# empymod/emg3d

Hardware: AMD Instinct MI355X
Metric: Mcells/s per multigrid cycle (higher is better)
Workload: dtype c128

## Files before the change

### emg3d_amd/_lib.py

```python
import ctypes
import os

import numpy as np

_HERE = os.path.dirname(os.path.abspath(__file__))
LIB_PATH = os.environ.get("EMG3D_HIP_LIB") or os.path.join(_HERE, "libemg3d_hip.so")
LAB_PATH = os.path.join(_HERE, "libemg3d_hip_lab.so")

c_i64 = ctypes.c_int64
c_int = ctypes.c_int
c_vp = ctypes.c_void_p
c_double = ctypes.c_double
c_dp = ctypes.POINTER(ctypes.c_double)

ABI_VERSION = 104

SIGNATURES = {
    "emg3d_hip_version": (c_int, []),
    "emg3d_hip_device_count": (c_int, [ctypes.POINTER(c_int)]),
    "emg3d_hip_set_device": (c_int, [c_int]),
    "emg3d_hip_device_info": (c_int, [c_int, ctypes.c_char_p, ctypes.POINTER(c_i64), ctypes.POINTER(c_int)]),
    "emg3d_hip_mem_info": (c_int, [c_int, ctypes.POINTER(c_i64), ctypes.POINTER(c_i64)]),
    "emg3d_hip_release_cached": (c_i64, []),
    "emg3d_hip_cached_bytes": (c_i64, []),
    "emg3d_hip_cached_bytes_on": (c_i64, [c_int]),
    "emg3d_mg_placement": (c_int, [c_vp, c_int, ctypes.POINTER(c_int), ctypes.POINTER(c_int), ctypes.POINTER(ctypes.c_float)]),
    "emg3d_amat_x": (c_int, [c_int, c_i64, c_i64, c_i64, c_vp, c_vp, c_vp, c_vp, c_vp, c_vp, c_vp, c_vp, c_vp]),
    "emg3d_get_h_field": (c_int, [c_int, c_i64, c_i64, c_i64, c_vp, c_vp, c_vp, c_vp, c_vp, c_vp, c_double, c_double]),
    "emg3d_gauss_seidel": (c_int, [c_int, c_int, c_i64, c_i64, c_i64, c_vp, c_vp, c_vp, c_vp, c_vp, c_vp,
                                   c_vp, c_vp, c_vp, c_int, c_int]),
    "emg3d_restrict": (c_int, [c_int, c_i64, c_i64, c_i64, c_i64, c_i64, c_i64, c_vp, c_vp, c_vp, c_int]),
    "emg3d_restrict_weights": (c_int, [c_vp, c_vp, c_vp, c_i64, c_vp, c_vp, c_vp, c_i64, c_vp, c_vp, c_vp]),
    "emg3d_solve": (c_int, [c_int, c_vp, c_vp, c_i64]),
    "emg3d_blocks_to_amat": (c_int, [c_int, c_vp, c_vp, c_i64, c_vp, c_vp, c_vp, c_i64, c_i64]),
    "emg3d_prolongation": (c_int, [c_int, c_i64, c_i64, c_i64, c_vp, c_vp, c_vp, c_vp, c_vp, c_vp, c_int]),
    "emg3d_restrict_model": (c_int, [c_int, c_i64, c_i64, c_i64, c_vp, c_vp, c_int]),
    "emg3d_sweep_plan": (c_int, [c_int, c_i64, c_i64, c_i64, c_int, c_int, c_int, c_int, ctypes.c_char_p, ctypes.POINTER(c_i64)]),
    "emg3d_mg_create": (c_int, [ctypes.POINTER(c_vp), c_int, c_i64, c_i64, c_i64, c_vp, c_vp, c_vp, c_vp,
                                c_vp, c_vp, c_vp, c_vp, c_int]),
    "emg3d_mg_destroy": (None, [c_vp]),
    "emg3d_mg_create_sv": (c_int, [ctypes.POINTER(c_vp), c_int, c_i64, c_i64, c_i64, c_vp, c_vp, c_vp, c_vp,
                                   c_vp, c_vp, c_vp, c_vp, c_double, c_double, c_int]),
    "emg3d_mg_create_vs": (c_int, [ctypes.POINTER(c_vp), c_int, c_i64, c_i64, c_i64, c_vp, c_vp, c_vp, c_vp,
                                   c_vp, c_vp, c_vp, c_vp, c_vp, c_double, c_double, c_int, c_int]),
    "emg3d_mg_create_vse": (c_int, [ctypes.POINTER(c_vp), c_int, c_i64, c_i64, c_i64, c_vp, c_vp, c_vp, c_vp,
                                    c_vp, c_vp, c_vp, c_vp, c_vp, c_vp, c_double, c_double, c_double, c_int, c_int]),
    "emg3d_mg_set_smu0_eps": (c_int, [c_vp, c_double, c_double, c_double]),
    "emg3d_mg_set_sfield_vector": (c_int, [c_vp, c_vp, c_double, c_double]),
    "emg3d_mg_set_sfield_dipole": (c_int, [c_vp, c_vp, c_vp, c_int, c_int, c_vp]),
    "emg3d_source_field": (c_int, [c_int, c_i64, c_i64, c_i64, c_vp, c_vp, c_vp, c_vp, c_vp, c_vp, c_int, c_vp, c_vp]),
    "emg3d_mg_prepare": (c_int, [c_vp, c_int, c_int]),
    "emg3d_mg_set_trace": (c_int, [c_vp, c_int]),
# ... 133 lines not shown
    return {"name": name.value.decode(), "total_mem": mem.value, "cu_count": cus.value}


def mem_info(device=0):
    fr, tot = c_i64(0), c_i64(0)
    check(load().emg3d_hip_mem_info(device, ctypes.byref(fr), ctypes.byref(tot)), "emg3d_hip_mem_info")
    return {"free": fr.value, "total": tot.value, "pooled": int(load().emg3d_hip_cached_bytes()),
            "pooled_on_device": int(load().emg3d_hip_cached_bytes_on(device))}


def sweep_plan(vnC, direction, dtype=np.complex128, ordering='colour', nsys=1, cu_count=0):
    name = ctypes.create_string_buffer(64)
    info = (c_i64 * 6)()
    check(load().emg3d_sweep_plan(dtype_code(dtype), int(vnC[0]), int(vnC[1]), int(vnC[2]), int(direction),
                                  1 if ordering == 'colour' else 0, int(nsys), int(cu_count), name, info), "emg3d_sweep_plan")
    return {"kernel": name.value.decode(), "lines_per_colour": info[0], "lines_per_wave": info[1], "rounds": info[2],
            "factor_kind": info[3], "split": bool(info[4]), "big_offsets": bool(info[5])}
```

### emg3d_amd/csrc/emg3d_hip.hip

```cpp
#include "../../include/emg3d_hip.h"

#include <cstring>
#include <new>

#include <chrono>
#include "mg.hpp"
#include "receivers.hpp"
#include "source.hpp"
#include "gradient.hpp"
#include "regrid.hpp"

#define EMG3D_HIP_VERSION EMG3D_HIP_ABI_VERSION

namespace {

template <class T>
MG<T>* as(emg3d_mg_t* mg) { return static_cast<MG<T>*>(reinterpret_cast<emg3d_mg*>(mg)); }

static int current_device() { int d = 0; if (hipGetDevice(&d) != hipSuccess) { (void)hipGetLastError(); d = 0; } return d; }

template <class T> static T scalar_of(double re, double im);
template <> double scalar_of<double>(double re, double) { return re; }
template <> c128 scalar_of<c128>(double re, double im) { return mk(re, im); }

// ... 481 lines not shown
    if (cu_count > 0) {
        m.cu_count = cu_count;
        m.tha_lds_state = 1; m.tha_lds_limit = 160 * 1024;
    } else m.device = current_device();
    m.order = order; m.nsys = nsys;
    m.lv0 = std::make_shared<Level<T>>();
    Level<T>& L = *m.lv0;
    L.nC[0] = nx; L.nC[1] = ny; L.nC[2] = nz;
    MG<T>::shape_level(L);
    i64 inf[6];
    m.plan_sweep(L, dir - 1, name, inf);
    for (int k = 0; k < 6; ++k) info[k] = inf[k];
    return 0;
}

extern "C" {

int emg3d_hip_version(void) { return EMG3D_HIP_VERSION; }

int64_t emg3d_hip_release_cached(void) { return (int64_t)DevicePool::get().release_all(); }
int64_t emg3d_hip_cached_bytes(void) { return (int64_t)DevicePool::get().bytes_held(); }
int64_t emg3d_hip_cached_bytes_on(int device) { return device < 0 ? 0 : (int64_t)DevicePool::get().bytes_held_on(device); }

int emg3d_hip_device_count(int* count) {
    HIP_TRY(hipGetDeviceCount(count));
    return 0;
}

int emg3d_hip_set_device(int device) {
    HIP_TRY(hipSetDevice(device));
// ... 76 lines not shown
    return dtype ? prolong_impl<c128>(nx, ny, nz, hx, hy, hz, origin, e, ce, sc_dir)
                 : prolong_impl<double>(nx, ny, nz, hx, hy, hz, origin, e, ce, sc_dir);
}

int emg3d_restrict_model(int is_complex, int64_t nx, int64_t ny, int64_t nz, void* cparam, const void* param,
                         int sc_dir) {
    return is_complex ? restrict_model_impl<c128>(nx, ny, nz, cparam, param, sc_dir)
                      : restrict_model_impl<double>(nx, ny, nz, cparam, param, sc_dir);
}

int emg3d_sweep_plan(int dtype, int64_t nx, int64_t ny, int64_t nz, int dir, int order, int nsys, int cu_count, char* name,
                     int64_t* info) {
    if (nx < 2 || ny < 2 || nz < 2 || dir < 1 || dir > 3 || order < 0 || order > 1 || nsys < 1 || nsys > 64 || !name || !info) return -2;
    return dtype ? sweep_plan_impl<c128>(nx, ny, nz, dir, order, nsys, cu_count, name, info)
                 : sweep_plan_impl<double>(nx, ny, nz, dir, order, nsys, cu_count, name, info);
}

int emg3d_mg_create(emg3d_mg_t** out, int dtype, int64_t nx, int64_t ny, int64_t nz, const double* hx,
                    const double* hy, const double* hz, const double* origin, const void* eta_x,
                    const void* eta_y, const void* eta_z, const double* zeta, int device) {
    if (!out) return -1;
    return dtype ? create_impl<c128>(out, 1, nx, ny, nz, hx, hy, hz, origin, eta_x, eta_y, eta_z, zeta, device)
                 : create_impl<double>(out, 0, nx, ny, nz, hx, hy, hz, origin, eta_x, eta_y, eta_z, zeta, device);
}

int emg3d_mg_create_sv(emg3d_mg_t** out, int dtype, int64_t nx, int64_t ny, int64_t nz, const double* hx,
                       const double* hy, const double* hz, const double* origin, const double* sv_x,
                       const double* sv_y, const double* sv_z, const double* zeta, double smu0_re,
                       double smu0_im, int device) {
    if (!out || !sv_x) return -1;
// ... 557 lines not shown
```

### emg3d_amd/csrc/mg.hpp

```cpp
#pragma once
#include <algorithm>
#include <cmath>
#include <cstdlib>
#include <cstring>
#include <map>
#include <memory>
#include <mutex>
#include <chrono>
#include <vector>

#include "common.hpp"
#include "smooth.hpp"
#include "stencil.hpp"
#include "smooth_qpl.hpp"
#include "smooth_qc.hpp"
#include "smooth_thm.hpp"
#include "smooth_tha.hpp"
#include "sweep_launch.hpp"

template <class T>
struct Level {
    i64 nC[3];
    i64 nE, nCells;
    FieldLayout fl;
// ... 6 lines not shown
    unsigned char* sflag[3] = {nullptr, nullptr, nullptr};
    bool sflag_valid[3] = {false, false, false};
    bool s_dense = false;
    bool zeta_sep = false;
    T *s = nullptr, *e = nullptr, *r = nullptr;
    T *eT = nullptr, *sT = nullptr;
    T* etaT[3] = {nullptr, nullptr, nullptr};
    double* zetaT = nullptr;
    bool sT_valid = false;
    FieldLayout flT;
    CellLayout clT;
    T *eW[2] = {nullptr, nullptr}, *sW[2] = {nullptr, nullptr};
    double* zetaW[2] = {nullptr, nullptr};
    bool sW_valid[2] = {false, false};
    int e_home = 0;
    T* fac[3] = {nullptr, nullptr, nullptr};
    void* qd[3][4] = {{nullptr, nullptr, nullptr, nullptr}, {nullptr, nullptr, nullptr, nullptr}, {nullptr, nullptr, nullptr, nullptr}};
    unsigned qdn[3][4] = {{0, 0, 0, 0}, {0, 0, 0, 0}, {0, 0, 0, 0}};
    i64 fac_lines[3] = {0, 0, 0};
    i64 fac_mid[3] = {0, 0, 0};
    int fac_kind[3] = {0, 0, 0};
};

struct Transfer {
    int sc = -1;
    int co[3] = {0, 0, 0};
    double* w[3][3] = {{nullptr, nullptr, nullptr}, {nullptr, nullptr, nullptr}, {nullptr, nullptr, nullptr}};
    int* pidx[3] = {nullptr, nullptr, nullptr};
    double* pwt[3] = {nullptr, nullptr, nullptr};
};
// ... 898 lines not shown
        a.xcd = xcd_map;
        a.tile = q_tile;
        {
            const int ax[3] = {a.L, a.P, a.Q};
            a.rs.ihL = a.ih[a.L]; a.rs.ihP = a.ih[a.P]; a.rs.ihQ = a.ih[a.Q];
            a.rs.hL = a.h[a.L]; a.rs.hP = a.h[a.P]; a.rs.hQ = a.h[a.Q];
            a.rs.nL = (unsigned)a.nC[a.L]; a.rs.slot0 = 0;
            a.rs.nP = (unsigned)a.nC[a.P]; a.rs.nQ = (unsigned)a.nC[a.Q];
            a.rs.csL = (unsigned)a.cl.st[a.L]; a.rs.csP = (unsigned)a.cl.st[a.P]; a.rs.csQ = (unsigned)a.cl.st[a.Q];
            for (int c = 0; c < 3; ++c) {
                a.rs.off[c] = (unsigned)a.fl.off[ax[c]];
                for (int d = 0; d < 3; ++d) a.rs.st[c][d] = (unsigned)a.fl.st[ax[c]][ax[d]];
            }
        }
        a.qd = nullptr; a.qdn = 0;
        a.qpl = 0; a.qM = 0; a.seg = 0; a.qlpw = 0;
        if (qpl(L, dir)) { int NW, M, seg; qpl_shape(L.nC[a.L], NW, M, seg); a.qpl = NW; a.qM = M; a.seg = seg; }
        a.tha = tha_helpers(L, dir);
        a.mode = 0; a.cP = a.cQ = 0; a.cntA = a.cntB = 0; a.t = a.jQ0 = a.cnt = 0;
        a.bt = sweep ? batch(L) : Batch();
    }

    bool q_on(const LineArgs<T>& a) const {
        return use_q >= 2 || (use_q == 1 && a.nA[0] * a.nB2[0] >= q_min_lines());
    }
    bool thm_on(const Level<T>& L, const LineArgs<T>& a) const { return twist_ok(L, a); }
    bool twist_ok(const Level<T>& L, const LineArgs<T>& a) const {
        if (q_on(a)) return false;
        if (!use_twist || !rp_fits(L) || L.nC[a.L] < 3) return false;
        const i64 nQ = L.nC[a.Q];
// ... 360 lines not shown
            L.eW[w] = cands[best];
            block_tag[cands[best]] = 1 + w;
            for (int k = 0; k < R.tries; ++k) if (k != best) release(cands[k]);
            moved |= best != 0;
            if (getenv("EMG3D_LOG_SETUP")) {
                fprintf(stderr, "[place] working copy %d (%s-lines, %.0f MB): kept candidate %d of %d;", w, dir == 0 ? "x" : dir == 1 ? "y" : "z",
                        (double)n * sizeof(T) / 1048576.0, best, R.tries);
                for (int k = 0; k < R.tries; ++k) fprintf(stderr, " %.3f", R.ms[k]);
                fprintf(stderr, " ms per sweep\n");
            }
        }
        if (moved) drop_graphs();
        check_launch();
    }

    void smooth_line(Level<T>& L, int dir, int nu, bool conv_in = true, bool conv_out = true) {
        if (nu <= 0) return;
        ensure_factor(L, dir);
        ensure_qdesc(L, dir);
        if (dry) { prepare_work(L, dir); return; }
        if (conv_in) to_work(L, dir);
        ensure_sflags(L, dir);
        LineArgs<T> a;
        line_args(L, dir, a, true);
        const bool big = q_big(L) && !rp_fits(L);
        const bool rp = rp_fits(L) || big;
        const i64 nP = L.nC[a.P], nQ = L.nC[a.Q];
        const i64 nB[2] = {(nQ - 0) / 2, (nQ - 1) / 2};
        int iback = 0;
        int last_c = -1;
        for (int it = 0; it < nu; ++it) {
            iback = 1 - iback;
            if (order == 1) {
                for (int ch = 0; ch < 4; ++ch) {
                    const int c = iback ? colour_perm_b[ch] : colour_perm[ch];
                    if (skip_idempotent && c == last_c) continue;
                    last_c = c;
                    a.mode = 0; a.cP = c & 1; a.cQ = c >> 1;
                    a.cntA = a.nA[a.cP]; a.cntB = nB[a.cQ];
                    a.rs.slot0 = (unsigned)a.base[c];
                    a.qd = L.qd[dir][c]; a.qdn = (L.qd[dir][c] ? L.qdn[dir][c] : 0u);
                    const i64 n = a.cntA * a.cntB;
                    if (n <= 0) continue;
// ... 62 lines not shown
                                       dim3(EMG_LINE_BLOCK), 0, stream, a);
                }
            }
        }
        if (hl) convert_field(L, L.eW[1], L.e, 1, true);
        check_launch();
    }

    void smoothing(Level<T>& L, int nu, int lr_dir) {
        const int lr = current_lr_dir(lr_dir, L.nC);
        if (lr == 0) smooth_point(L, nu);
        int dirs[3], nd = 0;
        if (lr == 1 || lr == 5 || lr == 6 || lr == 7) dirs[nd++] = 0;
        if (lr == 2 || lr == 4 || lr == 6 || lr == 7) dirs[nd++] = 1;
        if (lr == 3 || lr == 4 || lr == 5 || lr == 7) dirs[nd++] = 2;
        for (int k = 0; k < nd; ++k) {
            const bool in = (k == 0) || work_id(L, dirs[k - 1]) != work_id(L, dirs[k]);
            const bool out = (k == nd - 1) || work_id(L, dirs[k + 1]) != work_id(L, dirs[k]);
            smooth_line(L, dirs[k], nu, in, out);
        }
    }

    void residual(Level<T>& L, int mode, int slot) {
        ResidualArgs<T> a;
        for (int q = 0; q < 3; ++q) { a.nC[q] = L.nC[q]; a.eta[q] = L.eta[q]; a.h[q] = L.h[q]; a.ih[q] = L.ih[q]; }
        a.fl = L.fl; a.r = L.r; a.s = L.s; a.e = L.e; a.zeta = L.zeta; a.bt = batch(L);
        if (!dry && L.e_home == 1) {
            if (!L.sW_valid[1]) { convert_field(L, L.sW[1], L.s, 1, true); L.sW_valid[1] = true; }
            a.e = L.eW[1]; a.s = L.sW[1]; a.xs = 1;
        }
        const i64 plane = (L.nC[0] + 1) * (L.nC[1] + 1);
        const i64 cells = L.nC[0] * L.nC[1] * L.nC[2];
        const int kz = cells < res_zm_min ? 1 : res_kz ? res_kz : (cells * nsys >= ((i64)8 << 20) ? 8 : 4);
        const i64 nNz = L.nC[2] + 1;
// ... 209 lines not shown
```

### emg3d_amd/csrc/smooth.hpp

```cpp
#pragma once
#include "common.hpp"

#define EMG_LINE_BLOCK 64

template <class T>
struct LineArgs {
    int L, P, Q;
    i64 nC[3];
    FieldLayout fl;
    CellLayout cl;
    T* e;
    const T* s;
    const T* eta[3];
    const double* zeta;
    const double* h[3];
    const double* ih[3];
    int split;
    i64 mid;
    int xcd;
    int tile;
    struct Resolved {
        const double *ihL, *ihP, *ihQ;
        const double *hL, *hP, *hQ;
        unsigned nL, csL, csP, csQ;
// ... 5 lines not shown
    int qm;
    int qpl;
    int qM, seg;
    const unsigned char* sflag;
    int zsep;
    int qlpw;
    int tha;
    int fcomp;
    T* fac;
    const void* qd;
    unsigned qdn;
    i64 nLinesTot;
    i64 base[4];
    i64 nA[2];
    i64 nB2[2];
    int mode;
    int cP, cQ;
    i64 cntA, cntB;
    i64 t, jQ0, cnt;
};

template <class T>
__device__ __forceinline__ bool line_of_thread(const LineArgs<T>& a, i64& jP, i64& jQ) {
    const i64 idx = (i64)blockIdx.x * blockDim.x + threadIdx.x;
    if (a.mode == 0) {
        if (idx >= a.cntA * a.cntB) return false;
        const i64 b = idx / a.cntA, q = idx - b * a.cntA;
        jP = 1 + a.cP + 2 * q;
        jQ = 1 + a.cQ + 2 * b;
    } else {
// ... 1165 lines not shown
```

### emg3d_amd/csrc/smooth_qpl.hpp

```cpp
#pragma once
#include "smooth.hpp"


template <int K>
__device__ __forceinline__ double quad_bcast(double v) {
    constexpr int ctrl = K | (K << 2) | (K << 4) | (K << 6);
    int lo = __double2loint(v), hi = __double2hiint(v);
    lo = __builtin_amdgcn_update_dpp(0, lo, ctrl, 0xf, 0xf, false);
    hi = __builtin_amdgcn_update_dpp(0, hi, ctrl, 0xf, 0xf, false);
    return __hiloint2double(hi, lo);
}
template <int K>
__device__ __forceinline__ c128 quad_bcast(c128 v) { return mk(quad_bcast<K>(v.re), quad_bcast<K>(v.im)); }
__device__ __forceinline__ double quad_sum(double v) {
    int lo = __double2loint(v), hi = __double2hiint(v);
    double o = __hiloint2double(__builtin_amdgcn_update_dpp(0, hi, 0xb1, 0xf, 0xf, false),
                                __builtin_amdgcn_update_dpp(0, lo, 0xb1, 0xf, 0xf, false));
    v += o;
    lo = __double2loint(v); hi = __double2hiint(v);
    o = __hiloint2double(__builtin_amdgcn_update_dpp(0, hi, 0x4e, 0xf, 0xf, false),
                         __builtin_amdgcn_update_dpp(0, lo, 0x4e, 0xf, 0xf, false));
    return v + o;
}
__device__ __forceinline__ c128 quad_sum(c128 v) { return mk(quad_sum(v.re), quad_sum(v.im)); }
// ... 9 lines not shown
template <bool UP> __device__ __forceinline__ c128 row_shift4(c128 v) { return mk(row_shift4<UP>(v.re), row_shift4<UP>(v.im)); }
template <bool UP> __device__ __forceinline__ double lane_shift4(double v) { return UP ? __shfl_up(v, 4) : __shfl_down(v, 4); }
template <bool UP> __device__ __forceinline__ c128 lane_shift4(c128 v) { return mk(lane_shift4<UP>(v.re), lane_shift4<UP>(v.im)); }

template <class T>
__device__ __forceinline__ void qpl_args_burst(const LineArgs<T>& a) {
    asm volatile("" :: "s"(a.e), "s"(a.s), "s"(a.fac), "s"(a.zeta), "s"(a.rs.ihL), "s"(a.rs.ihP), "s"(a.rs.ihQ), "s"(a.bt.st),
                 "s"(a.bt.mask), "s"(a.bt.n), "s"(a.xcd), "s"(a.mode), "s"(a.cntA), "s"(a.cntB), "s"(a.cP), "s"(a.cQ), "s"(a.seg),
                 "s"(a.rs.nL), "s"(a.rs.csL), "s"(a.rs.csP), "s"(a.rs.csQ), "s"(a.rs.slot0), "s"(a.rs.off[0]), "s"(a.rs.off[1]),
                 "s"(a.rs.off[2]));
    asm volatile("" :: "s"(a.rs.st[0][0]), "s"(a.rs.st[0][1]), "s"(a.rs.st[0][2]), "s"(a.rs.st[1][0]), "s"(a.rs.st[1][1]),
                 "s"(a.rs.st[1][2]), "s"(a.rs.st[2][0]), "s"(a.rs.st[2][1]), "s"(a.rs.st[2][2]), "s"(a.t), "s"(a.jQ0), "s"(a.cnt),
                 "s"(a.rs.nP), "s"(a.rs.nQ), "s"(a.qd), "s"(a.qdn));
}

template <class T, int NW, int M, bool HL = false, int DM = 0, bool CH = false>
__global__ __launch_bounds__(64 * NW) void k_line_sweep_qpl(LineArgs<T> a) {
    static_assert(DM == 0 || (!HL && NW == 1), "descriptors: one wave per workgroup, colour order");
    static_assert(!CH || (NW == 1 && M == 1 && !HL), "chain form: lines inside one wave, one block per quad");
    constexpr int NQ = 16 * NW;
#ifdef EMG3D_LAB
    long long qts[7] = {0, 0, 0, 0, 0, 0, 0};
#define QPL_TS(i) do { if (a.tile & 512) { asm volatile("" ::: "memory"); qts[i] = (long long)__builtin_readcyclecounter(); asm volatile("" ::: "memory"); } } while (0)
#else
#define QPL_TS(i) do {} while (0)
#endif
    QPL_TS(0);
    qpl_args_burst(a);
    QPL_TS(1);
    const int tid = threadIdx.x;
    const int quad = tid >> 2, r = tid & 3;
    const int seg = a.seg;
    const int ch = quad & (seg - 1);
    const int lseg = __builtin_ctz((unsigned)seg);
    const int lpg = NQ >> lseg;
    typedef unsigned int u32;
    EMG_SWEEP_WG(a)
    __shared__ T xb[2][NQ][4][5];
    auto one = [&](const u32 gline, const u32 nlines, const u32 t_, const u32 jQ0_) {
    const bool live = gline < nlines;
    const int nL = (int)a.rs.nL;
    auto ld_d = [](const double* base, u32 idx) -> double { return *reinterpret_cast<const double*>(reinterpret_cast<const char*>(base) + idx * 8u); };
    auto ld_t = [](const T* base, u32 idx) -> T { return *reinterpret_cast<const T*>(reinterpret_cast<const char*>(base) + idx * (u32)sizeof(T)); };
    const T* __restrict__ e = (a.e + boff_);
    const T* __restrict__ s = (a.s + boff_);
    T Wr[M][5], W0[M][5];
    T b[M][5];
    double av[M][4], dv[M][4];
    bool lastb[M], inl[M];
    u32 dS[M], dS0[M];
    const u32 tix = (u32)wg * (64u * NW) + (u32)tid;
    constexpr int QD_U4 = 3, QD_D2 = 8;
    if constexpr (DM == 2) {
        const uint4* const q4 = reinterpret_cast<const uint4*>(a.qd);
        const emg_d2* const c2 = reinterpret_cast<const emg_d2*>(q4 + (size_t)(QD_U4 * M) * a.qdn);
        uint4 u[M][QD_U4];
        emg_d2 cf[M][QD_D2];
#pragma unroll
        for (int j = 0; j < M; ++j) {
#pragma unroll
            for (int k = 0; k < QD_U4; ++k) u[j][k] = q4[(u32)(QD_U4 * j + k) * a.qdn + tix];
#pragma unroll
            for (int k = 0; k < QD_D2; ++k) cf[j][k] = c2[(u32)(QD_D2 * j + k) * a.qdn + tix];
        }
        QPL_TS(2);
// ... 25 lines not shown
            dv[j][0] = cf[j][5].y; dv[j][1] = cf[j][6].x; dv[j][2] = cf[j][6].y; dv[j][3] = cf[j][7].x;
            T y = S[j];
#pragma unroll
            for (int t = 0; t < 6; ++t) cmac(y, E[j][t], cE[t]);
            const T bo = lastb[j] ? Zero<T>::v() : y;
            T part = E0[j] * cf[j][3].x;
            part = quad_sum(part);
            b[j][0] = S0[j] + part;
            b[j][1] = quad_bcast<0>(bo); b[j][2] = quad_bcast<1>(bo); b[j][3] = quad_bcast<2>(bo); b[j][4] = quad_bcast<3>(bo);
            if (!inl[j]) {
#pragma unroll
                for (int c = 0; c < 5; ++c) { Wr[j][c] = Zero<T>::v(); W0[j][c] = Zero<T>::v(); }
            }
        }
    } else {
    const u32 gidx = live ? gline : 0u;
    u32 jP, jQ;
    if (a.mode == 0) {
        const u32 cA = (u32)a.cntA;
        const u32 bq = gidx / cA, qq = gidx - bq * cA;
        jP = 1u + (u32)a.cP + 2u * qq;
        jQ = 1u + (u32)a.cQ + 2u * bq;
    } else {
        jQ = jQ0_ + gidx;
        jP = t_ - 2u * jQ;
    }
    const u32 slot = (a.mode == 0) ? a.rs.slot0 + gidx : (u32)line_slot(a, (i64)jP, (i64)jQ);
    const u32 csL = a.rs.csL, csP = a.rs.csP, csQ = a.rs.csQ;
    const double ihP[2] = {ld_d(a.rs.ihP, jP - 1u), ld_d(a.rs.ihP, jP)};
    const double ihQ[2] = {ld_d(a.rs.ihQ, jQ - 1u), ld_d(a.rs.ihQ, jQ)};
    const bool tp = r < 2;
    const int side = r & 1;
    const double sg = side ? -1.0 : 1.0;
    const u32 jA = tp ? jP : jQ, jB = tp ? jQ : jP;
    const u32 acell = jA - 1u + (u32)side;
    const u32 anode = side ? jA + 1u : jA - 1u;
    const u32 oLc = a.rs.off[0], oAc = tp ? a.rs.off[1] : a.rs.off[2], oBc = tp ? a.rs.off[2] : a.rs.off[1];
    const u32 sLL = a.rs.st[0][0];
    const u32 sLA = tp ? a.rs.st[0][1] : a.rs.st[0][2], sLB = tp ? a.rs.st[0][2] : a.rs.st[0][1];
    const u32 sAL = tp ? a.rs.st[1][0] : a.rs.st[2][0];
    const u32 sAA = tp ? a.rs.st[1][1] : a.rs.st[2][2], sAB = tp ? a.rs.st[1][2] : a.rs.st[2][1];
    const u32 sBL = tp ? a.rs.st[2][0] : a.rs.st[1][0];
    const u32 sBA = tp ? a.rs.st[2][1] : a.rs.st[1][2], sBB = tp ? a.rs.st[2][2] : a.rs.st[1][1];
    u32 ob[7], os[7];
    ob[0] = oAc + sAL + acell * sAA + jB * sAB;
    ob[1] = oLc + sLL + anode * sLA + jB * sLB;
    ob[2] = ob[1] - sLL;
    ob[3] = oBc + sBL + anode * sBA + jB * sBB;
    ob[4] = ob[3] - sBB;
    ob[5] = ob[0] + sAB;
    ob[6] = ob[0] - sAB;
    os[0] = sAL; os[1] = sLL; os[2] = sLL; os[3] = sBL; os[4] = sBL; os[5] = sAL; os[6] = sAL;
    const u32 sLP = a.rs.st[0][1], sLQ = a.rs.st[0][2];
    const u32 o0 = oLc + jP * sLP + jQ * sLQ;
    const u32 db0 = (r < 2) ? sLP : sLQ;
    const u32 ob0 = (r & 1) ? o0 - db0 : o0 + db0;
    const int type = tp ? 1 : 2;

    T E[M][6], S[M], E0[M], S0[M];
    u32 dE[M][6], dE0[M], dF[M];
    double f00[M], f10[M], f01[M], f11[M], n0[M], n1[M], ihl0[M], ihl1[M];
#pragma unroll
    for (int j = 0; j < M; ++j) {
        const int i = ch * M + j;
        const int ic = i < nL ? i : nL - 1;
        inl[j] = i < nL;
        lastb[j] = (ic == nL - 1);
        if constexpr (DM == 0) {
            const T* w = a.fac + ((i64)slot * (15 * (M * seg)) + ic);
#pragma unroll
            for (int c = 0; c < 5; ++c) W0[j][c] = w[(u32)(wpk(0, c) * (M * seg))];
#pragma unroll
// ... 6 lines not shown
            dF[j] = slot * (u32)(15 * (M * seg)) + (u32)ic;
        }
        const u32 cface = (jP - 1u) * csP + (jQ - 1u) * csQ + (u32)ic * csL;
        f00[j] = ld_d(a.zeta, cface); f10[j] = ld_d(a.zeta, cface + csP); f01[j] = ld_d(a.zeta, cface + csQ); f11[j] = ld_d(a.zeta, cface + csP + csQ);
        const u32 cnext = lastb[j] ? 0u : csL;
        const u32 pa = (type == 1) ? (u32)side * csP : (u32)side * csQ;
        const u32 pb = (type == 1) ? csQ : csP;
        n0[j] = ld_d(a.zeta, cface + cnext + pa); n1[j] = ld_d(a.zeta, cface + cnext + pa + pb);
        ihl0[j] = ld_d(a.rs.ihL, (u32)ic); ihl1[j] = ld_d(a.rs.ihL, (u32)(lastb[j] ? ic : ic + 1));
        const u32 ie = (u32)(lastb[j] ? (ic > 0 ? ic - 1 : 0) : ic);
#pragma unroll
        for (int t = 0; t < 6; ++t) dE[j][t] = ob[1 + t] + ie * os[1 + t];
        dS[j] = ob[0] + ie * os[0];
        dE0[j] = ob0 + (u32)ic * sLL;
        dS0[j] = o0 + (u32)ic * sLL;
        if constexpr (DM == 0) {
#pragma unroll
            for (int t = 0; t < 6; ++t) E[j][t] = ld_t(e, dE[j][t]);
            S[j] = ld_t(s, dS[j]);
            E0[j] = ld_t(e, dE0[j]);
            S0[j] = ld_t(s, dS0[j]);
        }
    }
    QPL_TS(2);
    const double kP[2] = {0.5 * ihP[0], 0.5 * ihP[1]};
    const double kQ[2] = {0.5 * ihQ[0], 0.5 * ihQ[1]};
    double Kc[6];
    {
        const double ihA = tp ? (side ? ihP[1] : ihP[0]) : (side ? ihQ[1] : ihQ[0]);
        const double kB0 = tp ? kQ[0] : kP[0], kB1 = tp ? kQ[1] : kP[1];
        const double ihB0 = tp ? ihQ[0] : ihP[0], ihB1 = tp ? ihQ[1] : ihP[1];
// ... 220 lines not shown
    }
    publish(p);
    sync();
#pragma unroll
    for (int k = 0; k < 4; ++k) v[k] = (ch + 1 < seg) ? xb[p][quad + 1][k][0] : Zero<T>::v();
    }
    QPL_TS(5);
    T* eo = (a.e + boff_);
#pragma unroll
    for (int j = M - 1; j >= 0; --j) {
        T x0 = z0[j], xr = zr[j];
#pragma unroll
        for (int l = 0; l < 4; ++l) { cmsc(x0, W0[j][l + 1], v[l]); cmsc(xr, Wr[j][l + 1], v[l]); }
        const int i = ch * M + j;
        if (live && inl[j]) {
            if (r == 0) eo[dS0[j]] = x0;
            if (!lastb[j]) eo[dS[j]] = xr;
        }
        if (j > 0) {
            const double ar = (r == 0) ? av[j][0] : (r == 1) ? av[j][1] : (r == 2) ? av[j][2] : av[j][3];
            const double dr = (r == 0) ? dv[j][0] : (r == 1) ? dv[j][1] : (r == 2) ? dv[j][2] : dv[j][3];
            T vr = x0 * ar;
            cmac(vr, xr, dr);
            v[0] = quad_bcast<0>(vr); v[1] = quad_bcast<1>(vr); v[2] = quad_bcast<2>(vr); v[3] = quad_bcast<3>(vr);
        }
    }
    QPL_TS(6);
    };

    if constexpr (!HL) {
        one((u32)wg * (u32)lpg + (u32)(quad >> lseg), (u32)((a.mode == 0) ? a.cntA * a.cntB : a.cnt), (u32)a.t, (u32)a.jQ0);
#ifdef EMG3D_LAB
        if ((a.tile & 512) && blockIdx.x == 0 && threadIdx.x == 0) {
            asm volatile("s_waitcnt vmcnt(0)" ::: "memory");
            const long long tend = (long long)__builtin_readcyclecounter();
            printf("[qpl<%d,%d> seg %d lines %lld] args %lld loads issued %lld loads in + coefficients %lld forward %lld backward %lld stores issued %lld stores done %lld (cycles after entry)\n",
                   NW, M, seg, (long long)(a.cntA * a.cntB), qts[1] - qts[0], qts[2] - qts[0], qts[3] - qts[0], qts[4] - qts[0], qts[5] - qts[0], qts[6] - qts[0], tend - qts[0]);
        }
#endif
    } else {
        const int nPm = (int)a.rs.nP - 1, nQm = (int)a.rs.nQ - 1;
        const int tmin = (int)a.t, tmax = (int)a.jQ0;
        for (int th = tmin; th <= tmax; ++th) {
            const int tt = a.cnt ? tmax - (th - tmin) : th;
            const int lo = tt - nPm;
// ... 15 lines not shown
```

### emg3d_amd/csrc/sweep_launch.hpp

```cpp
#pragma once
#include "smooth.hpp"
#include "stencil.hpp"

template <class T> void qc_launch(int stages, int lpw, bool zsep, bool big, dim3 grid, hipStream_t st, const LineArgs<T>& a);

template <class T> void thm_launch(int stages, int lpw, bool lifo, bool zsep, dim3 grid, hipStream_t st, const LineArgs<T>& a);
template <class T> void thm_lifo_attrs();

template <class T> void tha_launch(int helpers, bool zsep, dim3 grid, size_t dyn_lds, hipStream_t st, const LineArgs<T>& a);
template <class T> bool tha_attrs(int max_dyn_lds);

template <class T> void qpl_launch(int nw, int m, bool hl, int dm, bool chain, dim3 grid, hipStream_t st, const LineArgs<T>& a);

template <class T> void residual_launch(int mode, int kz, dim3 grid, hipStream_t st, const ResidualArgs<T>& a);
```

### emg3d_amd/csrc/sweep_qpl.hip

```cpp
#include "sweep_launch.hpp"
#ifndef EMG3D_UNIT_T
#define EMG3D_UNIT_T 2
#endif
#include "smooth_qpl.hpp"

template <class T, int NW, int M>
static void qpl_launch_c(dim3 grid, hipStream_t st, const LineArgs<T>& a) {
    hipLaunchKernelGGL((k_line_sweep_qpl<T, NW, M>), grid, dim3(64 * NW), 0, st, a);
}
template <class T, int NW>
static void qpl_launch_hl(dim3 grid, hipStream_t st, const LineArgs<T>& a) {
    hipLaunchKernelGGL((k_line_sweep_qpl<T, NW, 1, true>), grid, dim3(64 * NW), 0, st, a);
}
template <class T, int M>
static void qpl_launch_m(int nw, int dm, bool chain, dim3 grid, hipStream_t st, const LineArgs<T>& a) {
    if constexpr (M == 1) {
        if (chain && dm != 1 && nw == 1) {
            if (dm == 2) hipLaunchKernelGGL((k_line_sweep_qpl<T, 1, 1, false, 2, true>), grid, dim3(64), 0, st, a);
            else hipLaunchKernelGGL((k_line_sweep_qpl<T, 1, 1, false, 0, true>), grid, dim3(64), 0, st, a);
            return;
        }
    }
    if (dm == 1) hipLaunchKernelGGL((k_line_sweep_qpl<T, 1, M, false, 1>), grid, dim3(64), 0, st, a);
    else if (dm == 2) hipLaunchKernelGGL((k_line_sweep_qpl<T, 1, M, false, 2>), grid, dim3(64), 0, st, a);
    else if (nw == 1) qpl_launch_c<T, 1, M>(grid, st, a);
    else if (nw == 2) qpl_launch_c<T, 2, M>(grid, st, a);
    else if (nw == 4) qpl_launch_c<T, 4, M>(grid, st, a);
    else qpl_launch_c<T, 8, M>(grid, st, a);
}
template <class T>
void qpl_launch(int nw, int m, bool hl, int dm, bool chain, dim3 grid, hipStream_t st, const LineArgs<T>& a) {
    if (hl) {
        if (nw == 1) qpl_launch_hl<T, 1>(grid, st, a);
        else if (nw == 2) qpl_launch_hl<T, 2>(grid, st, a);
        else if (nw == 4) qpl_launch_hl<T, 4>(grid, st, a);
        else qpl_launch_hl<T, 8>(grid, st, a);
    } else if (m == 2) qpl_launch_m<T, 2>(nw, dm, false, grid, st, a);
    else qpl_launch_m<T, 1>(nw, dm, chain, grid, st, a);
}
#if EMG3D_UNIT_T != 1
template void qpl_launch<double>(int, int, bool, int, bool, dim3, hipStream_t, const LineArgs<double>&);
#endif
#if EMG3D_UNIT_T != 0
template void qpl_launch<c128>(int, int, bool, int, bool, dim3, hipStream_t, const LineArgs<c128>&);
#endif
```

### include/emg3d_hip.h

```cpp
#ifndef EMG3D_HIP_H
#define EMG3D_HIP_H

#include <stdint.h>

#ifdef __cplusplus
extern "C" {
#endif

#define EMG3D_HIP_ABI_VERSION 104
int emg3d_hip_version(void);
int emg3d_hip_device_count(int* count);
int emg3d_hip_set_device(int device);
int emg3d_hip_device_info(int device, char* name, int64_t* total_mem, int* cu_count);
int emg3d_hip_mem_info(int device, int64_t* free_bytes, int64_t* total_bytes);

int64_t emg3d_hip_release_cached(void);
int64_t emg3d_hip_cached_bytes(void);
int64_t emg3d_hip_cached_bytes_on(int device);


int emg3d_amat_x(int dtype, int64_t nx, int64_t ny, int64_t nz, void* r, const void* e,
                 const void* eta_x, const void* eta_y, const void* eta_z, const double* zeta,
                 const double* hx, const double* hy, const double* hz);

// ... 15 lines not shown

int emg3d_solve(int dtype, void* amat, void* bvec, int64_t n);

int emg3d_blocks_to_amat(int dtype, void* amat, void* bvec, int64_t n, const void* middle,
                         const double* left, const void* rhs, int64_t im, int64_t nC);

int emg3d_prolongation(int dtype, int64_t nx, int64_t ny, int64_t nz, const double* hx,
                       const double* hy, const double* hz, const double* origin, void* e,
                       const void* ce, int sc_dir);

int emg3d_restrict_model(int is_complex, int64_t nx, int64_t ny, int64_t nz, void* cparam,
                         const void* param, int sc_dir);

int emg3d_sweep_plan(int dtype, int64_t nx, int64_t ny, int64_t nz, int dir, int order, int nsys, int cu_count, char* name,
                     int64_t* info);

typedef struct emg3d_mg emg3d_mg_t;

int emg3d_mg_create(emg3d_mg_t** out, int dtype, int64_t nx, int64_t ny, int64_t nz,
                    const double* hx, const double* hy, const double* hz, const double* origin,
                    const void* eta_x, const void* eta_y, const void* eta_z, const double* zeta,
                    int device);
int emg3d_mg_create_sv(emg3d_mg_t** out, int dtype, int64_t nx, int64_t ny, int64_t nz, const double* hx,
                       const double* hy, const double* hz, const double* origin, const double* sv_x,
                       const double* sv_y, const double* sv_z, const double* zeta, double smu0_re,
                       double smu0_im, int device);

int emg3d_mg_create_vs(emg3d_mg_t** out, int dtype, int64_t nx, int64_t ny, int64_t nz, const double* hx,
                       const double* hy, const double* hz, const double* origin, const double* sigma_x,
                       const double* sigma_y, const double* sigma_z, const double* vol, const double* zeta,
// ... 98 lines not shown
```

Measured before the change: 249.7.

## Fuse all colour passes of a line smoothing into one LDS-resident slab kernel

Adds a colour-loop variant of the chained quad-per-line sweep kernel. Each workgroup loads a slab of the field (with a halo sized from the colour sequence) into dynamic LDS, runs every colour pass of the nu iterations inside the kernel with workgroup barriers, and writes its owned slab to a ping-pong buffer. This replaces many separate per-colour launches and their global-memory round trips. It is enabled by default for eligible levels when consecutive directions both qualify, and it costs an extra field buffer, redundant halo computation, and low workgroup counts on small grids.

New measurement: 252.3, median of 6. +1.1%, better.

```diff
diff --git a/emg3d_amd/_lib.py b/emg3d_amd/_lib.py
--- a/emg3d_amd/_lib.py
+++ b/emg3d_amd/_lib.py
@@ -36,6 +36,7 @@
     "emg3d_prolongation": (c_int, [c_int, c_i64, c_i64, c_i64, c_vp, c_vp, c_vp, c_vp, c_vp, c_vp, c_int]),
     "emg3d_restrict_model": (c_int, [c_int, c_i64, c_i64, c_i64, c_vp, c_vp, c_int]),
     "emg3d_sweep_plan": (c_int, [c_int, c_i64, c_i64, c_i64, c_int, c_int, c_int, c_int, ctypes.c_char_p, ctypes.POINTER(c_i64)]),
+    "emg3d_colour_loop_plan": (c_int, [c_int, c_i64, c_i64, c_i64, c_int, c_int, c_int, ctypes.POINTER(c_i64)]),
     "emg3d_mg_create": (c_int, [ctypes.POINTER(c_vp), c_int, c_i64, c_i64, c_i64, c_vp, c_vp, c_vp, c_vp,
                                 c_vp, c_vp, c_vp, c_vp, c_int]),
     "emg3d_mg_destroy": (None, [c_vp]),
@@ -199,5 +200,18 @@
     info = (c_i64 * 6)()
     check(load().emg3d_sweep_plan(dtype_code(dtype), int(vnC[0]), int(vnC[1]), int(vnC[2]), int(direction),
                                   1 if ordering == 'colour' else 0, int(nsys), int(cu_count), name, info), "emg3d_sweep_plan")
-    return {"kernel": name.value.decode(), "lines_per_colour": info[0], "lines_per_wave": info[1], "rounds": info[2],
-            "factor_kind": info[3], "split": bool(info[4]), "big_offsets": bool(info[5])}
+    out = {"kernel": name.value.decode(), "lines_per_colour": info[0], "lines_per_wave": info[1], "rounds": info[2],
+           "factor_kind": info[3], "split": bool(info[4]), "big_offsets": bool(info[5])}
+    loop = colour_loop_plan(vnC, direction, 2, dtype, cu_count) if ordering == 'colour' else None
+    out.update({"colour_loop": bool(loop and loop["on"]), "slab_width": loop["slab_width"] if loop and loop["on"] else 0,
+                "halo": loop["halo"] if loop and loop["on"] else []})
+    return out
+
+
+def colour_loop_plan(vnC, direction, nu=2, dtype=np.complex128, cu_count=0):
+    info = (c_i64 * 32)()
+    check(load().emg3d_colour_loop_plan(dtype_code(dtype), int(vnC[0]), int(vnC[1]), int(vnC[2]), int(direction), int(nu),
+                                        int(cu_count), info), "emg3d_colour_loop_plan")
+    n = int(info[4])
+    return {"on": bool(info[0]), "slab_axis": int(info[1]), "slab_width": int(info[2]), "workgroups": int(info[3]),
+            "lds_bytes": int(info[5]), "colours": [int(info[6 + p]) for p in range(n)], "halo": [int(info[18 + p]) for p in range(n)]}
diff --git a/emg3d_amd/csrc/emg3d_hip.hip b/emg3d_amd/csrc/emg3d_hip.hip
--- a/emg3d_amd/csrc/emg3d_hip.hip
+++ b/emg3d_amd/csrc/emg3d_hip.hip
@@ -519,6 +519,31 @@
     return 0;
 }
 
+template <class T>
+static int colour_loop_plan_impl(i64 nx, i64 ny, i64 nz, int dir, int nu, int cu_count, int64_t* info) {
+    MG<T> m;
+    if (cu_count > 0) m.cu_count = cu_count;
+    else m.device = current_device();
+    m.order = 1; m.nsys = 1;
+    m.lv0 = std::make_shared<Level<T>>();
+    Level<T>& L = *m.lv0;
+    L.nC[0] = nx; L.nC[1] = ny; L.nC[2] = nz;
+    MG<T>::shape_level(L);
+    LineArgs<T> a;
+    m.line_args(L, dir - 1, a, true);
+    int col[12], h[12];
+    const int np = m.colour_seq(nu, col, 12);
+    if (np <= 0) return -2;
+    const int ax = L.nC[a.Q] > L.nC[a.P] ? 1 : 0;
+    MG<T>::colour_loop_halo(col, np, ax, h);
+    size_t lds = 0;
+    const bool on = m.colour_loop_plan(L, nu, a, lds);
+    for (int k = 0; k < 32; ++k) info[k] = 0;
+    info[0] = on; info[1] = ax; info[2] = m.cloop_w; info[3] = on ? a.cl_ng : 0; info[4] = np; info[5] = (int64_t)lds;
+    for (int p = 0; p < np; ++p) { info[6 + p] = col[p]; info[18 + p] = h[p]; }
+    return 0;
+}
+
 extern "C" {
 
 int emg3d_hip_version(void) { return EMG3D_HIP_VERSION; }
@@ -625,6 +650,12 @@
     if (nx < 2 || ny < 2 || nz < 2 || dir < 1 || dir > 3 || order < 0 || order > 1 || nsys < 1 || nsys > 64 || !name || !info) return -2;
     return dtype ? sweep_plan_impl<c128>(nx, ny, nz, dir, order, nsys, cu_count, name, info)
                  : sweep_plan_impl<double>(nx, ny, nz, dir, order, nsys, cu_count, name, info);
+}
+
+int emg3d_colour_loop_plan(int dtype, int64_t nx, int64_t ny, int64_t nz, int dir, int nu, int cu_count, int64_t* info) {
+    if (nx < 2 || ny < 2 || nz < 2 || dir < 1 || dir > 3 || nu < 1 || nu > 3 || !info) return -2;
+    return dtype ? colour_loop_plan_impl<c128>(nx, ny, nz, dir, nu, cu_count, info)
+                 : colour_loop_plan_impl<double>(nx, ny, nz, dir, nu, cu_count, info);
 }
 
 int emg3d_mg_create(emg3d_mg_t** out, int dtype, int64_t nx, int64_t ny, int64_t nz, const double* hx,
diff --git a/emg3d_amd/csrc/mg.hpp b/emg3d_amd/csrc/mg.hpp
--- a/emg3d_amd/csrc/mg.hpp
+++ b/emg3d_amd/csrc/mg.hpp
@@ -44,6 +44,7 @@
     double* zetaW[2] = {nullptr, nullptr};
     bool sW_valid[2] = {false, false};
     int e_home = 0;
+    T* eB = nullptr;
     T* fac[3] = {nullptr, nullptr, nullptr};
     void* qd[3][4] = {{nullptr, nullptr, nullptr, nullptr}, {nullptr, nullptr, nullptr, nullptr}, {nullptr, nullptr, nullptr, nullptr}};
     unsigned qdn[3][4] = {{0, 0, 0, 0}, {0, 0, 0, 0}, {0, 0, 0, 0}};
@@ -972,6 +973,8 @@
             }
         }
         a.qd = nullptr; a.qdn = 0;
+        a.e2 = nullptr; a.cl_np = 0; a.cl_ax = 0; a.cl_w = a.cl_ng = a.cl_hmax = a.cl_wp = 0;
+        for (int p = 0; p < 12; ++p) a.cl_col[p] = a.cl_h[p] = 0;
         a.qpl = 0; a.qM = 0; a.seg = 0; a.qlpw = 0;
         if (qpl(L, dir)) { int NW, M, seg; qpl_shape(L.nC[a.L], NW, M, seg); a.qpl = NW; a.qM = M; a.seg = seg; }
         a.tha = tha_helpers(L, dir);
@@ -1362,10 +1365,79 @@
         check_launch();
     }
 
-    void smooth_line(Level<T>& L, int dir, int nu, bool conv_in = true, bool conv_out = true) {
+    int use_cloop = (int)LAB_ENV("EMG3D_COLOUR_LOOP", 1);
+    int cloop_w = (int)LAB_ENV("EMG3D_COLOUR_LOOP_W", 2);
+    int colour_seq(int nu, int* col, int cap) const {
+        int n = 0, iback = 0, last_c = -1;
+        for (int it = 0; it < nu; ++it) {
+            iback = 1 - iback;
+            for (int ch = 0; ch < 4; ++ch) {
+                const int c = iback ? colour_perm_b[ch] : colour_perm[ch];
+                if (skip_idempotent && c == last_c) continue;
+                last_c = c;
+                if (n >= cap) return -1;
+                col[n++] = c;
+            }
+        }
+        return n;
+    }
+    static void colour_loop_halo(const int* col, int np, int ax, int* h) {
+        for (int p = 0; p < np; ++p) h[p] = 0;
+        for (int b = 0; b < 2; ++b) {
+            const int n0 = 64 + b, n1 = 64 + b;
+            int lo = 2 * n0, hi = 2 * n1 - 1;
+            for (int p = np - 1; p >= 0; --p) {
+                const int par = (1 + ((ax ? col[p] >> 1 : col[p]) & 1)) & 1;
+                int jl = lo / 2;
+                if ((jl & 1) != par) ++jl;
+                int jh = (hi + 1) / 2;
+                if ((jh & 1) != par) --jh;
+                h[p] = std::max(h[p], std::max(n0 - jl, jh - (n1 - 1)));
+                lo = std::min(lo, 2 * jl - 2);
+                hi = std::max(hi, 2 * jh + 2);
+            }
+        }
+    }
+    bool colour_loop_plan(const Level<T>& L, int nu, LineArgs<T>& a, size_t& lds) const {
+        a.cl_np = 0;
+        lds = 0;
+        if (!use_cloop || order != 1 || a.qpl != 1 || a.qM != 1 || a.seg > qpl_chain_seg || a.split || cloop_w < 1) return false;
+        int col[12], h[12];
+        const int np = colour_seq(nu, col, 12);
+        if (np <= 0) return false;
+        const int ax = L.nC[a.Q] > L.nC[a.P] ? 1 : 0;
+        const i64 nS = L.nC[ax ? a.Q : a.P];
+        const i64 ng = std::max<i64>(1, (nS + 1) / cloop_w), wmax = (nS + 1) - (ng - 1) * cloop_w;
+        colour_loop_halo(col, np, ax, h);
+        int hmax = 0;
+        for (int p = 0; p < np; ++p) hmax = std::max(hmax, h[p]);
+        const i64 across = ax ? a.nA[0] : a.nB2[0];
+        i64 widest = 0;
+        for (int p = 0; p < np; ++p) widest = std::max(widest, ((wmax + 2 * h[p]) / 2 + 1) * across);
+        const i64 lpw = 16 / a.seg, waves = (widest + lpw - 1) / lpw;
+        const i64 S = simds(), per_cu = std::max<i64>(1, S / std::max(1, cu_count));
+        if (waves > std::min<i64>(4, per_cu) || ng * waves > S) return false;
+        const i64 wp = wmax + 2 * hmax + 2;
+        const i64 nL = L.nC[a.L], nP = L.nC[a.P], nQ = L.nC[a.Q];
+        const i64 cells = ax ? nL * (nP + 1) + (nL + 1) * nP + (nL + 1) * (nP + 1) : nL * (nQ + 1) + (nL + 1) * (nQ + 1) + (nL + 1) * nQ;
+        lds = (size_t)(cells * wp) * sizeof(T);
+        if (lds > 64 * 1024) { lds = 0; return false; }
+        a.cl_np = np; a.cl_ax = ax; a.cl_w = cloop_w; a.cl_ng = (int)ng; a.cl_hmax = hmax; a.cl_wp = (int)wp;
+        for (int p = 0; p < np; ++p) { a.cl_col[p] = (unsigned char)col[p]; a.cl_h[p] = (unsigned char)h[p]; }
+        return true;
+    }
+    bool colour_loop_on(Level<T>& L, int dir, int nu) {
+        LineArgs<T> a;
+        line_args(L, dir, a, true);
+        size_t lds;
+        return colour_loop_plan(L, nu, a, lds);
+    }
+
+    void smooth_line(Level<T>& L, int dir, int nu, bool conv_in = true, bool conv_out = true, int loop = 0) {
         if (nu <= 0) return;
         ensure_factor(L, dir);
         ensure_qdesc(L, dir);
+        if (loop && !L.eB) L.eB = dalloc<T>(nsys * L.nE);
         if (dry) { prepare_work(L, dir); return; }
         if (conv_in) to_work(L, dir);
         ensure_sflags(L, dir);
@@ -1375,6 +1447,18 @@
         const bool rp = rp_fits(L) || big;
         const i64 nP = L.nC[a.P], nQ = L.nC[a.Q];
         const i64 nB[2] = {(nQ - 0) / 2, (nQ - 1) / 2};
+        size_t lds = 0;
+        if (loop && L.eB && colour_loop_plan(L, nu, a, lds)) {
+            a.e = (loop == 1) ? L.e : L.eB;
+            a.e2 = (loop == 1) ? L.eB : L.e;
+            if (log_launches) fprintf(stderr, "[sweep] nC %lld %lld %lld L %d colour loop: %d passes, %d workgroups, %zu B LDS\n", (long long)a.nC[0],
+                                      (long long)a.nC[1], (long long)a.nC[2], a.L, a.cl_np, a.cl_ng, lds);
+            note_kernel("k_line_sweep_qpl_chain", a.qpl, a.qM);
+            if (!broken) qpl_loop_launch<T>(bgrid(qpl_grid(a.cl_ng)), lds, stream, a);
+            if (conv_out) from_work(L, dir);
+            check_launch();
+            return;
+        }
         int iback = 0;
         int last_c = -1;
         for (int it = 0; it < nu; ++it) {
@@ -1467,10 +1551,17 @@
         if (lr == 1 || lr == 5 || lr == 6 || lr == 7) dirs[nd++] = 0;
         if (lr == 2 || lr == 4 || lr == 6 || lr == 7) dirs[nd++] = 1;
         if (lr == 3 || lr == 4 || lr == 5 || lr == 7) dirs[nd++] = 2;
+        int loop[3] = {0, 0, 0};
+        if (order == 1 && use_cloop && nd > 1) {
+            bool ok[3] = {false, false, false};
+            for (int k = 0; k < nd; ++k) ok[k] = colour_loop_on(L, dirs[k], nu);
+            for (int k = 0; k + 1 < nd; ++k)
+                if (ok[k] && ok[k + 1]) { loop[k] = 1; loop[k + 1] = 2; ++k; }
+        }
         for (int k = 0; k < nd; ++k) {
             const bool in = (k == 0) || work_id(L, dirs[k - 1]) != work_id(L, dirs[k]);
             const bool out = (k == nd - 1) || work_id(L, dirs[k + 1]) != work_id(L, dirs[k]);
-            smooth_line(L, dirs[k], nu, in, out);
+            smooth_line(L, dirs[k], nu, in, out, loop[k]);
         }
     }
 
diff --git a/emg3d_amd/csrc/smooth.hpp b/emg3d_amd/csrc/smooth.hpp
--- a/emg3d_amd/csrc/smooth.hpp
+++ b/emg3d_amd/csrc/smooth.hpp
@@ -43,6 +43,12 @@
     i64 base[4];
     i64 nA[2];
     i64 nB2[2];
+    T* e2;
+    int cl_np;
+    int cl_ax;
+    int cl_w, cl_ng;
+    int cl_hmax, cl_wp;
+    unsigned char cl_col[12], cl_h[12];
     int mode;
     int cP, cQ;
     i64 cntA, cntB;
diff --git a/emg3d_amd/csrc/smooth_qpl.hpp b/emg3d_amd/csrc/smooth_qpl.hpp
--- a/emg3d_amd/csrc/smooth_qpl.hpp
+++ b/emg3d_amd/csrc/smooth_qpl.hpp
@@ -47,10 +47,11 @@
                  "s"(a.rs.nP), "s"(a.rs.nQ), "s"(a.qd), "s"(a.qdn));
 }
 
-template <class T, int NW, int M, bool HL = false, int DM = 0, bool CH = false>
+template <class T, int NW, int M, bool HL = false, int DM = 0, bool CH = false, bool CL = false>
 __global__ __launch_bounds__(64 * NW) void k_line_sweep_qpl(LineArgs<T> a) {
     static_assert(DM == 0 || (!HL && NW == 1), "descriptors: one wave per workgroup, colour order");
-    static_assert(!CH || (NW == 1 && M == 1 && !HL), "chain form: lines inside one wave, one block per quad");
+    static_assert(!CH || ((NW == 1 || CL) && M == 1 && !HL), "chain form: lines inside one wave, one block per quad");
+    static_assert(!CL || (CH && DM == 0), "colour loop: chain form, indices computed in the kernel");
     constexpr int NQ = 16 * NW;
 #ifdef EMG3D_LAB
     long long qts[7] = {0, 0, 0, 0, 0, 0, 0};
@@ -69,9 +70,14 @@
     const int lpg = NQ >> lseg;
     typedef unsigned int u32;
     EMG_SWEEP_WG(a)
-    __shared__ T xb[2][NQ][4][5];
+    __shared__ T xb[2][CL ? 1 : NQ][4][5];
+    extern __shared__ __attribute__((aligned(16))) char qpl_dyn_lds[];
+    T* const fw = reinterpret_cast<T*>(qpl_dyn_lds);
+    u32 clP = (u32)a.cP, clQ = (u32)a.cQ, clA = (u32)a.cntA, clS0 = a.rs.slot0;
+    bool clLive = true;
+    u32 w0 = 0, loff[3] = {0, 0, 0}, lst[3][3] = {{0, 0, 0}, {0, 0, 0}, {0, 0, 0}};
     auto one = [&](const u32 gline, const u32 nlines, const u32 t_, const u32 jQ0_) {
-    const bool live = gline < nlines;
+    const bool live = CL ? clLive : gline < nlines;
     const int nL = (int)a.rs.nL;
     auto ld_d = [](const double* base, u32 idx) -> double { return *reinterpret_cast<const double*>(reinterpret_cast<const char*>(base) + idx * 8u); };
     auto ld_t = [](const T* base, u32 idx) -> T { return *reinterpret_cast<const T*>(reinterpret_cast<const char*>(base) + idx * (u32)sizeof(T)); };
@@ -82,6 +88,7 @@
     double av[M][4], dv[M][4];
     bool lastb[M], inl[M];
     u32 dS[M], dS0[M];
+    u32 lS[M], lS0[M];
     const u32 tix = (u32)wg * (64u * NW) + (u32)tid;
     constexpr int QD_U4 = 3, QD_D2 = 8;
     if constexpr (DM == 2) {
@@ -137,18 +144,18 @@
             }
         }
     } else {
-    const u32 gidx = live ? gline : 0u;
+    const u32 gidx = (CL || live) ? gline : 0u;
     u32 jP, jQ;
-    if (a.mode == 0) {
-        const u32 cA = (u32)a.cntA;
+    if (CL || a.mode == 0) {
+        const u32 cA = CL ? clA : (u32)a.cntA;
         const u32 bq = gidx / cA, qq = gidx - bq * cA;
-        jP = 1u + (u32)a.cP + 2u * qq;
-        jQ = 1u + (u32)a.cQ + 2u * bq;
+        jP = 1u + (CL ? clP : (u32)a.cP) + 2u * qq;
+        jQ = 1u + (CL ? clQ : (u32)a.cQ) + 2u * bq;
     } else {
         jQ = jQ0_ + gidx;
         jP = t_ - 2u * jQ;
     }
-    const u32 slot = (a.mode == 0) ? a.rs.slot0 + gidx : (u32)line_slot(a, (i64)jP, (i64)jQ);
+    const u32 slot = CL ? clS0 + gidx : (a.mode == 0) ? a.rs.slot0 + gidx : (u32)line_slot(a, (i64)jP, (i64)jQ);
     const u32 csL = a.rs.csL, csP = a.rs.csP, csQ = a.rs.csQ;
     const double ihP[2] = {ld_d(a.rs.ihP, jP - 1u), ld_d(a.rs.ihP, jP)};
     const double ihQ[2] = {ld_d(a.rs.ihQ, jQ - 1u), ld_d(a.rs.ihQ, jQ)};
@@ -179,6 +186,26 @@
     const u32 db0 = (r < 2) ? sLP : sLQ;
     const u32 ob0 = (r & 1) ? o0 - db0 : o0 + db0;
     const int type = tp ? 1 : 2;
+    u32 lb[7], lo0 = 0, lob0 = 0;
+    if constexpr (CL) {
+        const u32 fP = a.cl_ax ? jP : jP - w0, fQ = a.cl_ax ? jQ - w0 : jQ;
+        const u32 fA = tp ? fP : fQ, fB = tp ? fQ : fP;
+        const u32 facell = fA - 1u + (u32)side, fanode = side ? fA + 1u : fA - 1u;
+        const u32 lLc = loff[0], lAc = tp ? loff[1] : loff[2], lBc = tp ? loff[2] : loff[1];
+        const u32 tAL = tp ? lst[1][0] : lst[2][0], tAA = tp ? lst[1][1] : lst[2][2], tAB = tp ? lst[1][2] : lst[2][1];
+        const u32 tLA = tp ? lst[0][1] : lst[0][2], tLB = tp ? lst[0][2] : lst[0][1];
+        const u32 tBL = tp ? lst[2][0] : lst[1][0], tBA = tp ? lst[2][1] : lst[1][2], tBB = tp ? lst[2][2] : lst[1][1];
+        lb[0] = lAc + tAL + facell * tAA + fB * tAB;
+        lb[1] = lLc + lst[0][0] + fanode * tLA + fB * tLB;
+        lb[2] = lb[1] - lst[0][0];
+        lb[3] = lBc + tBL + fanode * tBA + fB * tBB;
+        lb[4] = lb[3] - tBB;
+        lb[5] = lb[0] + tAB;
+        lb[6] = lb[0] - tAB;
+        lo0 = lLc + fP * lst[0][1] + fQ * lst[0][2];
+        const u32 ldb0 = (r < 2) ? lst[0][1] : lst[0][2];
+        lob0 = (r & 1) ? lo0 - ldb0 : lo0 + ldb0;
+    }
 
     T E[M][6], S[M], E0[M], S0[M];
     u32 dE[M][6], dE0[M], dF[M];
@@ -215,7 +242,17 @@
         dS[j] = ob[0] + ie * os[0];
         dE0[j] = ob0 + (u32)ic * sLL;
         dS0[j] = o0 + (u32)ic * sLL;
-        if constexpr (DM == 0) {
+        if constexpr (CL) {
+            const u32 los[7] = {lst[1 + (tp ? 0 : 1)][0], lst[0][0], lst[0][0], lst[2 - (tp ? 0 : 1)][0], lst[2 - (tp ? 0 : 1)][0],
+                                lst[1 + (tp ? 0 : 1)][0], lst[1 + (tp ? 0 : 1)][0]};
+#pragma unroll
+            for (int t = 0; t < 6; ++t) E[j][t] = fw[lb[1 + t] + ie * los[1 + t]];
+            lS[j] = lb[0] + ie * los[0];
+            lS0[j] = lo0 + (u32)ic * lst[0][0];
+            S[j] = ld_t(s, dS[j]);
+            E0[j] = fw[lob0 + (u32)ic * lst[0][0]];
+            S0[j] = ld_t(s, dS0[j]);
+        } else if constexpr (DM == 0) {
 #pragma unroll
             for (int t = 0; t < 6; ++t) E[j][t] = ld_t(e, dE[j][t]);
             S[j] = ld_t(s, dS[j]);
@@ -466,8 +503,13 @@
         for (int l = 0; l < 4; ++l) { cmsc(x0, W0[j][l + 1], v[l]); cmsc(xr, Wr[j][l + 1], v[l]); }
         const int i = ch * M + j;
         if (live && inl[j]) {
-            if (r == 0) eo[dS0[j]] = x0;
-            if (!lastb[j]) eo[dS[j]] = xr;
+            if constexpr (CL) {
+                if (r == 0) fw[lS0[j]] = x0;
+                if (!lastb[j]) fw[lS[j]] = xr;
+            } else {
+                if (r == 0) eo[dS0[j]] = x0;
+                if (!lastb[j]) eo[dS[j]] = xr;
+            }
         }
         if (j > 0) {
             const double ar = (r == 0) ? av[j][0] : (r == 1) ? av[j][1] : (r == 2) ? av[j][2] : av[j][3];
@@ -480,7 +522,71 @@
     QPL_TS(6);
     };
 
-    if constexpr (!HL) {
+    if constexpr (CL) {
+        const u32 nS = a.cl_ax ? a.rs.nQ : a.rs.nP;
+        if (wg >= a.cl_ng) return;
+        const int n0 = (int)wg * a.cl_w, n1 = (wg + 1 == a.cl_ng) ? (int)nS + 1 : n0 + a.cl_w;
+        w0 = (u32)max(0, n0 - a.cl_hmax - 1);
+        const int ds = 1 + a.cl_ax;
+        const u32 nn[3] = {a.rs.nL, a.rs.nP, a.rs.nQ};
+        u32 ext[3][3], full[3], total = 0;
+#pragma unroll
+        for (int c = 0; c < 3; ++c) {
+#pragma unroll
+            for (int d = 0; d < 3; ++d) ext[c][d] = nn[d] + (c == d ? 0u : 1u);
+            full[c] = ext[c][ds];
+            ext[c][ds] = (u32)a.cl_wp;
+            lst[c][0] = 1u; lst[c][1] = ext[c][0]; lst[c][2] = ext[c][0] * ext[c][1];
+            loff[c] = total;
+            total += ext[c][0] * ext[c][1] * ext[c][2];
+        }
+        auto locate = [&](u32 i, u32& g, u32& ps, int& cc) {
+            const int c = i >= loff[2] ? 2 : i >= loff[1] ? 1 : 0;
+            u32 l = i - loff[c];
+            const u32 i0 = l % ext[c][0];
+            l /= ext[c][0];
+            const u32 i1 = l % ext[c][1], i2 = l / ext[c][1];
+            const u32 p1 = ds == 1 ? i1 + w0 : i1, p2 = ds == 2 ? i2 + w0 : i2;
+            ps = ds == 1 ? p1 : p2;
+            g = a.rs.off[c] + i0 * a.rs.st[c][0] + p1 * a.rs.st[c][1] + p2 * a.rs.st[c][2];
+            cc = c;
+        };
+        const T* __restrict__ ea = a.e + boff_;
+        for (u32 i = (u32)tid; i < total; i += 64u * NW) {
+            u32 g, ps;
+            int c;
+            locate(i, g, ps, c);
+            fw[i] = ps < full[c] ? ea[g] : Zero<T>::v();
+        }
+        __syncthreads();
+        for (int p = 0; p < a.cl_np; ++p) {
+            const int c = a.cl_col[p], h = a.cl_h[p];
+            clP = (u32)(c & 1); clQ = (u32)(c >> 1); clA = (u32)a.nA[clP]; clS0 = (u32)a.base[c];
+            const int cs = (int)(a.cl_ax ? clQ : clP);
+            int lo = max(1, n0 - h);
+            const int hi = min((int)nS - 1, n1 - 1 + h);
+            if ((lo - 1 - cs) & 1) ++lo;
+            const int ns = hi >= lo ? (hi - lo) / 2 + 1 : 0;
+            const int nt = a.cl_ax ? (int)clA : (int)a.nB2[clQ];
+            const int nl = ns * nt;
+            for (int b0 = 0; b0 < nl; b0 += lpg) {
+                const int li0 = b0 + (quad >> lseg);
+                clLive = li0 < nl;
+                const int li = clLive ? li0 : 0;
+                const u32 ks = (u32)(lo + 2 * (li % ns)), kt = (u32)(li / ns);
+                const u32 qq = a.cl_ax ? kt : (ks - 1u - clP) / 2u, bq = a.cl_ax ? (ks - 1u - clQ) / 2u : kt;
+                one(bq * clA + qq, 0u, 0u, 0u);
+            }
+            __syncthreads();
+        }
+        T* __restrict__ eb = a.e2 + boff_;
+        for (u32 i = (u32)tid; i < total; i += 64u * NW) {
+            u32 g, ps;
+            int c;
+            locate(i, g, ps, c);
+            if ((int)ps >= n0 && (int)ps < n1 && ps < full[c]) eb[g] = fw[i];
+        }
+    } else if constexpr (!HL) {
         one((u32)wg * (u32)lpg + (u32)(quad >> lseg), (u32)((a.mode == 0) ? a.cntA * a.cntB : a.cnt), (u32)a.t, (u32)a.jQ0);
 #ifdef EMG3D_LAB
         if ((a.tile & 512) && blockIdx.x == 0 && threadIdx.x == 0) {
diff --git a/emg3d_amd/csrc/sweep_launch.hpp b/emg3d_amd/csrc/sweep_launch.hpp
--- a/emg3d_amd/csrc/sweep_launch.hpp
+++ b/emg3d_amd/csrc/sweep_launch.hpp
@@ -11,5 +11,6 @@
 template <class T> bool tha_attrs(int max_dyn_lds);
 
 template <class T> void qpl_launch(int nw, int m, bool hl, int dm, bool chain, dim3 grid, hipStream_t st, const LineArgs<T>& a);
+template <class T> void qpl_loop_launch(dim3 grid, size_t dyn_lds, hipStream_t st, const LineArgs<T>& a);
 
 template <class T> void residual_launch(int mode, int kz, dim3 grid, hipStream_t st, const ResidualArgs<T>& a);
diff --git a/emg3d_amd/csrc/sweep_qpl.hip b/emg3d_amd/csrc/sweep_qpl.hip
--- a/emg3d_amd/csrc/sweep_qpl.hip
+++ b/emg3d_amd/csrc/sweep_qpl.hip
@@ -38,9 +38,15 @@
     } else if (m == 2) qpl_launch_m<T, 2>(nw, dm, false, grid, st, a);
     else qpl_launch_m<T, 1>(nw, dm, chain, grid, st, a);
 }
+template <class T>
+void qpl_loop_launch(dim3 grid, size_t dyn_lds, hipStream_t st, const LineArgs<T>& a) {
+    hipLaunchKernelGGL((k_line_sweep_qpl<T, 4, 1, false, 0, true, true>), grid, dim3(256), dyn_lds, st, a);
+}
 #if EMG3D_UNIT_T != 1
+template void qpl_loop_launch<double>(dim3, size_t, hipStream_t, const LineArgs<double>&);
 template void qpl_launch<double>(int, int, bool, int, bool, dim3, hipStream_t, const LineArgs<double>&);
 #endif
 #if EMG3D_UNIT_T != 0
+template void qpl_loop_launch<c128>(dim3, size_t, hipStream_t, const LineArgs<c128>&);
 template void qpl_launch<c128>(int, int, bool, int, bool, dim3, hipStream_t, const LineArgs<c128>&);
 #endif
diff --git a/include/emg3d_hip.h b/include/emg3d_hip.h
--- a/include/emg3d_hip.h
+++ b/include/emg3d_hip.h
@@ -53,6 +53,7 @@
 
 int emg3d_sweep_plan(int dtype, int64_t nx, int64_t ny, int64_t nz, int dir, int order, int nsys, int cu_count, char* name,
                      int64_t* info);
+int emg3d_colour_loop_plan(int dtype, int64_t nx, int64_t ny, int64_t nz, int dir, int nu, int cu_count, int64_t* info);
 
 typedef struct emg3d_mg emg3d_mg_t;
 
```
